# Gaeric/bevy-hikari

Measured on AMD Instinct MI355X. Metric: Mrays/sec + ms/frame @1080p 1spp; cornell & city scenes, 1/2/4/8 GPU, higher is better.
Workload: dtype f32

## Files before the change

### bevy-hikari_amd/csrc/hk_device.h

```cpp
#pragma once

#include <hip/hip_runtime.h>
#include <stdint.h>

#include "../../include/hk_math.h"
#include "../../include/hk_types.h"
#include "../../include/hikari_amd.h"
#include "../../include/hk_texture.h"

namespace hk {

struct f2 {
    float x, y;
};
struct f3 {
    float x, y, z;
};
struct f4 {
    float x, y, z, w;
};
#define HKD __device__ __forceinline__
HKD f2 mk2(float x, float y) { return f2{x, y}; }
HKD f3 mk3(float x, float y, float z) { return f3{x, y, z}; }
HKD f4 mk4(float x, float y, float z, float w) { return f4{x, y, z, w}; }
// ... 80 lines not shown
    const hk_node* asset_nodes;
    const hk_alias_entry* alias_table;
    const hk_instance* instances;
    const hk_node* instance_nodes;
    const hk_material* materials;
    const hk_node* emissive_nodes;
    const hk_emissive* emissives;
    uint32_t n_instances, n_instance_nodes, n_materials, n_emissive_nodes;
    const float4* blas_wide;
    const float4* tlas_wide;
    uint32_t bytes[SCENE_ARRAYS];
    const hk_texture_desc* textures;
    const uint32_t* texels;
    const float* texture_lut;
    uint32_t n_textures;
};

constexpr uint32_t LDS_SCENE_MAX = 32768;
constexpr uint32_t LDS_WORKGROUP_MAX = 65536;
enum : int { PLAN_LIGHT = 0, PLAN_GBUFFER = 1 };
__host__ __device__ constexpr bool plan_has(int plan, int k)
{
    return plan == PLAN_LIGHT ? k < 9 : (k == 0 || k == 1 || k == 4 || k == 9 || k == 10);
}
__host__ __device__ inline uint32_t stage_bytes(const uint32_t* bytes, int plan)
{
    uint32_t total = 0;
    for (int k = 0; k < 11; ++k)
        if (plan_has(plan, k)) total += (bytes[k] + 15u) & ~15u;
    return total;
// ... 631 lines not shown
{
    f4 r = mat4_mul(in.model, mk4(p.x, p.y, p.z, 1.0f));
    if (r.w == 1.0f) return mk3(r.x, r.y, r.z);
    return mk3(r.x / r.w, r.y / r.w, r.z / r.w);
}
HKD f3 local_to_world_normal(const hk_instance& in, f3 n)
{
    const float* m = in.inverse_transpose_model;
    f3 r;
    r.x = (m[0] * n.x + m[4] * n.y) + m[8] * n.z;
    r.y = (m[1] * n.x + m[5] * n.y) + m[9] * n.z;
    r.z = (m[2] * n.x + m[6] * n.y) + m[10] * n.z;
    return normalize(r);
}

constexpr int LANE_SLOTS = 5;
#ifdef HK_LANE_STATS
extern __device__ unsigned long long hk_lane_stats_dev[2 * LANE_SLOTS];
template <int SLOT = 0>
struct LaneStats {
    unsigned long long act = 0, its = 0;
    HKD void tick()
    {
        const unsigned long long m = __ballot(1);
        if ((uint32_t)__builtin_ctzll(m) == (threadIdx.x & 63u)) {
            act += (unsigned long long)__builtin_popcountll(m);
            its += 1;
        }
    }
    HKD ~LaneStats()
    {
        if (its) {
            atomicAdd(&hk_lane_stats_dev[2 * SLOT], act);
            atomicAdd(&hk_lane_stats_dev[2 * SLOT + 1], its);
        }
    }
};
#define HK_LANE_STATS_DECL LaneStats<0> lane_stats_
#define HK_LANE_STATS_TICK lane_stats_.tick()
#define HK_STAGE_STATS_DECL LaneStats<1> stage1_; LaneStats<2> stage2_; LaneStats<3> stage3_; LaneStats<4> stage4_
#define HK_STAGE_TICK(k) stage##k##_.tick()
#else
#define HK_LANE_STATS_DECL
#define HK_LANE_STATS_TICK
#define HK_STAGE_STATS_DECL
#define HK_STAGE_TICK(k)
#endif

template <bool ANY_HIT = true>
HKD Hit traverse_top(const Scene& sc, const Ray& ray, float max_distance, float early_distance, uint32_t exclude)
{
    Hit hit;
    hit.uv = mk2(0.0f, 0.0f);
    hit.distance = max_distance;
    hit.instance_index = HK_U32_MAX;
    hit.primitive_index = HK_U32_MAX;
    const hk_node* nodes = sc.instance_nodes;
    uint32_t count = sc.n_instance_nodes, index = 0u;
    Ray tr = ray;
    uint32_t top = 0u;
    uint32_t prim_offset = 0u, cur_instance = 0u;
    bool in_bottom = false, intersected = false;
    HK_LANE_STATS_DECL;
    while (index < count) {
        HK_LANE_STATS_TICK;
// ... 31 lines not shown
            }
        } else {
            const uint32_t instance_index = leaf_entry - HK_BVH_LEAF_FLAG;
            if (leaf_pass && (!ANY_HIT || instance_index != exclude)) {
                const hk_instance& in = sc.instances[instance_index];
                const uint32_t bot_count = in.mesh.node[1];
                prim_offset = in.mesh.primitive;
                cur_instance = instance_index;
                intersected = false;
                if (bot_count > 0u) {
                    in_bottom = true;
                    top = index;
                    nodes = sc.asset_nodes + in.mesh.node[0];
                    count = bot_count;
                    index = 0u;
                    tr.origin = world_to_local_point(in, ray.origin);
                    tr.direction = world_to_local_dir(in, ray.direction);
                    tr.inv_direction = inv(tr.direction);
                }
            }
        }
    }
    return hit;
}
HKD Hit traverse_top_closest(const Scene& sc, const Ray& ray)
{
    return traverse_top<false>(sc, ray, HK_F32_MAX, 0.0f, DONT_EXCLUDE);
}

constexpr int GB_STACK = 64;
constexpr int GB_STACK_LDS = 16;
constexpr int GB_DEEP_LDS = 8;
template <bool SHALLOW, int LVL = GB_STACK_LDS>
struct GbStackT {
    uint2* lds;
    uint32_t node[SHALLOW ? 1 : GB_STACK - LVL];
    float t[SHALLOW ? 1 : GB_STACK - LVL];
    int sp;
// ... 557 lines not shown
```

### bevy-hikari_amd/csrc/hk_kernels.hip

```cpp
#include <stdlib.h>
#include <mutex>
#include <type_traits>

#include "hk_device.h"
#include "hk_launch.h"

namespace hk {

#ifdef HK_LANE_STATS
__device__ unsigned long long hk_lane_stats_dev[2 * LANE_SLOTS];
#endif
bool lane_stats_take(unsigned long long out[2 * LANE_SLOTS], hipStream_t st)
{
#ifdef HK_LANE_STATS
    unsigned long long zero[2 * LANE_SLOTS] = {};
    if (hipStreamSynchronize(st) != hipSuccess) return false;
    if (hipMemcpyFromSymbol(out, HIP_SYMBOL(hk_lane_stats_dev), sizeof(zero)) != hipSuccess) return false;
    return hipMemcpyToSymbol(HIP_SYMBOL(hk_lane_stats_dev), zero, sizeof(zero)) == hipSuccess;
#else
    (void)st;
    for (int k = 0; k < 2 * LANE_SLOTS; ++k) out[k] = 0;
    return false;
#endif
}
// ... 639 lines not shown
}

template <bool VD, bool VE, int PARK>
HKD void fused_direct_pixel(const FrameArgs& A, const Scene& sc, const ChannelArgs& C0, const ChannelArgs& C1,
                            const DirectPixel& P, uint32_t& n_top, uint32_t& n_emitter)
{
    const uint32_t bg = bg_elide(C0, P.idx, P.pd.w < HK_F32_EPSILON);
    if (bg == BG_SKIP_OWN) {
        store_background_pair(C1, P.idx);
    } else if (bg == BG_STORE) {
        Surface surface;
        direct_body<false, true, VD, PARK>(A, sc, C0, P, n_top, n_emitter, &surface);
        direct_body<true, false, VE, PARK>(A, sc, C1, P, n_top, n_emitter, nullptr, &surface);
    }
}
template <bool LDS, bool VD, bool VE>
HKD void direct_fused_kernel(FrameArgs A, ChannelArgs C0, ChannelArgs C1)
{
    int32_t x, y;
    const bool active = tile_pixel<TRACE_ORDER>(A.F, A.F.s[0], A.F.s_row0, A.F.s_rows, x, y);
    PixelTexels tex;
    if (active) tex = load_pixel_texels(A, x, y);
    Scene sc;
    if constexpr (LDS) sc = stage_scene<PLAN_LIGHT>(A.sc, hk_lds_scene);
    else sc = A.sc;
    uint32_t n_top = 0, n_emitter = 0;
    if (active) fused_direct_pixel<VD, VE, !LDS>(A, sc, C0, C1, direct_pixel_of(A, x, y, tex), n_top, n_emitter);
    finish_counts(A, x, y, n_top, n_emitter);
}
template <bool LDS, bool VD, bool VE>
__global__ __launch_bounds__(256) void k_direct_fused(FrameArgs A, ChannelArgs C0, ChannelArgs C1)
{
    direct_fused_kernel<LDS, VD, VE>(A, C0, C1);
}
template <bool LDS, bool VD, bool VE = false>
__global__ __launch_bounds__(256) __attribute__((amdgpu_waves_per_eu(4, 8))) void k_direct_fused_w4(FrameArgs A, ChannelArgs C0,
                                                                                                   ChannelArgs C1)
{
    direct_fused_kernel<LDS, VD, VE>(A, C0, C1);
}

constexpr uint32_t CW_LONG_NODES = 16u;
constexpr int CW_WORDS = 10;
static_assert(CW_WORDS <= PARK_WORDS, "the batch rows fit the park columns");
HKD float* cw_area()
{
    __shared__ float cw[CW_WORDS * 256];
    return cw;
}
struct WalkRows {
    float* lds;
    uint32_t col;
    HKD float& operator[](int k) const { return lds[k * 256 + col]; }
    HKD uint32_t bits(int k) const { return __float_as_uint(lds[k * 256 + col]); }
// ... 535 lines not shown
template <bool MULTI, int STAGE = IND_ALL>
HKD bool indirect_body(const FrameArgs& A, const Scene& sc, const ChannelArgs& C, int32_t x, int32_t y, uint32_t& n_top,
                       uint32_t& n_emitter, const WfArgs* W = nullptr, uint32_t* key = nullptr, IndStash* stash = nullptr,
                       const PixelTexels* tex = nullptr)
{
    IndirectState I;
    bool ret;
    if (!indirect_begin<MULTI, STAGE>(A, sc, C, x, y, n_top, n_emitter, W, key, I, ret, stash, tex)) return ret;
    Hit sh;
    if (!MULTI && I.shadow)
        sh = traverse_top(sc, I.B.ray, I.B.cand.max_distance, I.B.cand.min_distance, I.B.cand.emissive_instance);
    indirect_end<MULTI>(A, sc, C, I, sh, stash);
    return true;
}

template <bool MULTI, bool LDS, bool CS = false>
__global__ __launch_bounds__(256) void k_indirect(FrameArgs A, ChannelArgs C)
{
    int32_t x, y;
    const bool active = tile_pixel<TRACE_ORDER>(A.F, A.F.s[0], A.F.s_row0, A.F.s_rows, x, y);
    constexpr bool PRE = !MULTI && !LDS && !CS;
    PixelTexels tex;
    if (PRE && active) tex = load_pixel_texels(A, x, y);
    Scene sc = A.sc;
    if constexpr (LDS) {
        sc = stage_scene<PLAN_LIGHT>(A.sc, hk_lds_scene);
    }
    uint32_t n_top = 0, n_emitter = 0;
    if constexpr (CS && !MULTI) {
        IndirectState I;
        bool ret = false;
        const bool live = active && indirect_begin<false>(A, sc, C, x, y, n_top, n_emitter, nullptr, nullptr, I, ret);
        Hit sh;
        compact_top_walks(sc, cw_area(), live && I.shadow, I.B.ray, I.B.cand.max_distance, I.B.cand.min_distance,
                          I.B.cand.emissive_instance, sh);
        if (live) indirect_end<false>(A, sc, C, I, sh);
    } else if (active) {
        __shared__ IndStash stash;
        indirect_body<MULTI>(A, sc, C, x, y, n_top, n_emitter, nullptr, nullptr, &stash, PRE ? &tex : nullptr);
    }
    finish_counts(A, x, y, n_top, n_emitter);
}
// ... 911 lines not shown
            if (emissive_lit) hipLaunchKernelGGL((k_direct<true, false, LDS, VAL>), g, dim3(256), lds, st, A, C);
            else if (big) hipLaunchKernelGGL((k_direct_lit_w4<LDS, VAL>), g, dim3(256), lds, st, A, C);
            else hipLaunchKernelGGL((k_direct<false, true, LDS, VAL>), g, dim3(256), lds, st, A, C);
        },
        lds != 0u, val);
}
template <bool LDS>
static void launch_fused_v(const FrameArgs& A, const ChannelArgs& C0, const ChannelArgs& C1, bool vd, bool ve, dim3 g,
                           uint32_t lds, hipStream_t st)
{
    const bool w4 = A.opt.fused_w4 != 0;
    if (!LDS && w4 && !ve && (A.opt.compact_emitter || A.opt.compact_shadow)) {
        dispatch([&](auto VD, auto CS) { hipLaunchKernelGGL((k_direct_fused_cw<VD, CS>), g, dim3(256), lds, st, A, C0, C1); },
                 vd, A.opt.compact_shadow != 0);
    } else if (w4 && (!LDS || !ve)) {
        dispatch([&](auto VD, auto VE) { hipLaunchKernelGGL((k_direct_fused_w4<LDS, VD, VE>), g, dim3(256), lds, st, A, C0, C1); },
                 vd, ve);
    } else {
        dispatch([&](auto VD, auto VE) { hipLaunchKernelGGL((k_direct_fused<LDS, VD, VE>), g, dim3(256), lds, st, A, C0, C1); },
                 vd, ve);
    }
}
void launch_direct_fused(const FrameArgs& A, const ChannelArgs& C0, const ChannelArgs& C1, hipStream_t st)
{
    dim3 g = tiles(A.F, A.F.s[0], A.F.s_rows);
    const uint32_t lds = lds_plan_bytes(A, PLAN_LIGHT, true);
    const bool vd = validation_frame(A.F.number, A.F.direct_validate_interval);
    const bool ve = validation_frame(A.F.number, A.F.emissive_validate_interval);
    if (lds) launch_fused_v<true>(A, C0, C1, vd, ve, g, lds, st);
    else launch_fused_v<false>(A, C0, C1, vd, ve, g, 0, st);
}
static uint32_t persist_grid(const void* kernel, uint32_t lds, const Frame& F)
// ... 31 lines not shown
}
void launch_indirect(const FrameArgs& A, const ChannelArgs& C, bool multi, hipStream_t st)
{
    dim3 g = tiles(A.F, A.F.s[0], A.F.s_rows);
    const uint32_t lds = lds_plan_bytes(A, PLAN_LIGHT, true);
    if (A.opt.persistent_indirect) {
        dispatch(
            [&](auto M, auto L) {
                const dim3 pg(persist_grid((const void*)k_indirect_persist<M, L>, lds, A.F));
                hipLaunchKernelGGL((k_indirect_persist<M, L>), pg, dim3(256), lds, st, A, C);
            },
            multi, lds != 0u);
        return;
    }
    dispatch(
        [&](auto L) {
            if (multi) hipLaunchKernelGGL((k_indirect<true, L>), g, dim3(256), lds, st, A, C);
            else if (A.opt.compact_shadow) hipLaunchKernelGGL((k_indirect<false, L, true>), g, dim3(256), lds, st, A, C);
            else hipLaunchKernelGGL((k_indirect<false, L>), g, dim3(256), lds, st, A, C);
        },
        lds != 0u);
}
uint32_t indirect_stash_bytes() { return (uint32_t)sizeof(IndStash); }
static_assert(LDS_SCENE_MAX + sizeof(IndStash) <= LDS_WORKGROUP_MAX, "staged scene + stash exceed a workgroup's LDS");
bool light_lds_direct(const FrameArgs& A) { return lds_plan_bytes(A, PLAN_LIGHT, false) != 0u; }
void launch_light_merged(const FrameArgs& A, const ChannelArgs& C0, const ChannelArgs& C1, const ChannelArgs& C2,
                         hipStream_t st)
{
    dim3 g = tiles(A.F, A.F.s[0], A.F.s_rows);
    g.z = 2u;
    const uint32_t scene = lds_plan_bytes(A, PLAN_LIGHT, true);
    const bool vd = validation_frame(A.F.number, A.F.direct_validate_interval);
    const bool ve = validation_frame(A.F.number, A.F.emissive_validate_interval);
    const uint32_t park = (vd || ve) ? (uint32_t)(PARK_WORDS * 256 * sizeof(float)) : 0u;
    const uint32_t ind = scene + (uint32_t)sizeof(IndStash);
    const uint32_t lds = ind > park ? ind : park;
// ... 251 lines not shown
```

### bevy-hikari_amd/csrc/hk_runtime.hip

```cpp
#include <hip/hip_runtime.h>

#include <algorithm>
#include <array>
#include <cmath>
#include <cstdio>
#include <cstring>
#include <map>
#include <set>
#include <string>
#include <vector>

#include "../../include/hikari_amd.h"
#include "hk_launch.h"

using namespace hk;

namespace {
constexpr int32_t BAND_HALO = 40;
constexpr size_t COUNTER_SPAN = (size_t)COUNTER_SHARDS * COUNTER_STRIDE;
constexpr size_t COUNTER_BYTES = 3 * COUNTER_SPAN * sizeof(unsigned long long);
constexpr size_t PERSIST_BYTES = (size_t)PERSIST_KINDS * PERSIST_LINES * PERSIST_LINE * sizeof(unsigned long long);

struct TimedLaunch {
    const char* name;
    hipEvent_t start, stop;
};

// ... 10 lines not shown
    OPT_SPATIAL_VIEW,
    OPT_BAND_FULL_WINDOWS,
    OPT_LEAF_COLLAPSE,
    OPT_GBUFFER_REUSE,
    OPT_LDS_SCENE,
    OPT_GBUFFER_STACK_FULL,
    OPT_GBUFFER_DEEP,
    OPT_GBUFFER_LDS_MAX_PX,
    OPT_DIRECT_W4_MIN_PX,
    OPT_FUSED_W4,
    OPT_PERSISTENT_INDIRECT,
    OPT_COMPACT_EMITTER,
    OPT_COMPACT_SHADOW,
    OPT_FSR_TILED,
    OPT_PRESENT_RUN,
    OPT_COUNT
};
struct OptDef {
    const char* key;
    double def, lo, hi;
};
constexpr OptDef OPTS[OPT_COUNT] = {
    {"pipeline_min_px", 1.2e6, 0.0, 1e12}, {"pipeline_heavy_min_px", 0.0, 0.0, 1e12},
    {"gbuffer_pipeline", 1, 0, 1},         {"tail_pipeline", 1, 0, 1},
    {"channel_streams", 1, 0, 1},          {"fuse", 1, 0, 1},              {"fuse_min_px", 1048576.0, 0.0, 1e12},
    {"merge", -1, -1, 1},                  {"bg_elision", 1, 0, 1},        {"spatial_view_planes", 1, 0, 1},
    {"band_full_windows", 0, 0, 1},        {"leaf_collapse", 1, 0, 1},     {"gbuffer_reuse", 1, 0, 1},
    {"lds_scene", 1, 0, 2},                {"gbuffer_stack_full", 0, 0, 1}, {"gbuffer_deep", 0, 0, 1},
    {"gbuffer_lds_max_px", 6e5, 0.0, 1e12},
    {"direct_w4_min_px", 4e5, 0.0, 1e12},  {"fused_w4", 1, 0, 1},          {"persistent_indirect", 0, 0, 1},
    {"compact_emitter", 0, 0, 1},          {"compact_shadow", 0, 0, 1},    {"fsr_tiled", 1, 0, 1},
    {"present_run", 1, 0, 1},
};

struct GSlot {
    float4* position = nullptr;
    uint32_t* normal = nullptr;
    float2* depth_gradient = nullptr;
    float2* instance_material = nullptr;
    float4* velocity_uv = nullptr;
    uint2* albedo = nullptr;
};

struct ScheduleState {
    bool gb_pending = false;
    bool gb_serial = true;
    bool post_pending = false;
// ... 153 lines not shown
        uint32_t vertex_need;
        uint32_t depth;
        uint32_t used = 0;
    };
    std::vector<MeshSlice> meshes;
    size_t cap[9] = {};
    size_t collapse_cap = 0;
    std::vector<float> emissive;
    uint32_t* blas_aux = nullptr;
    void* mesh_scratch = nullptr;
    size_t mesh_bytes = 0;
    float* prev_models = nullptr;
    bool models_dirty = false;
    bool velocity_zero = true;
    bool has_scene = false;
    uchar4* noise = nullptr;
    bool has_noise = false;
    hk_texture_desc* tex_desc = nullptr;
    uint32_t* texels = nullptr;
    float* tex_lut = nullptr;
    uint32_t n_textures = 0;

    uint32_t S[2] = {0, 0}, s[2] = {0, 0};
    float ratio = 1.0f;
    int32_t S_row0 = 0, S_rows = 0, s_row0 = 0, s_rows = 0;
    int32_t core_row0 = 0, core_rows = 0;
    int32_t halo = BAND_HALO;
    int32_t stripe_n = 0, stripe_k = 0;
    bool albedo_fresh = false;
    bool sized = false;
// ... 209 lines not shown
{
    if (!c->event_pool.empty()) {
        hipEvent_t e = c->event_pool.back();
        c->event_pool.pop_back();
        return e;
    }
    hipEvent_t e = nullptr;
    (void)hipEventCreate(&e);
    return e;
}

void lane_stats_account(hk_ctx* c, const char* name, hipStream_t st)
{
    unsigned long long v[2 * LANE_SLOTS];
    if (!lane_stats_take(v, st)) return;
    static const char* const stage[LANE_SLOTS] = {"", "/neighbour", "/march_tap", "/record_tests", "/merge"};
    for (int slot = 0; slot < LANE_SLOTS; ++slot) {
        if (!v[2 * slot + 1]) continue;
        const std::string key = std::string(name) + stage[slot];
        size_t k = 0;
        for (; k < c->lane_names.size(); ++k)
            if (c->lane_names[k] == key) break;
        if (k == c->lane_names.size()) {
            c->lane_names.push_back(key);
            c->lane_act.push_back(0);
            c->lane_its.push_back(0);
        }
        c->lane_act[k] += v[2 * slot];
        c->lane_its[k] += v[2 * slot + 1];
    }
}
// ... 64 lines not shown
    A.sc.instances = (const hk_instance*)c->buf[4];
    A.sc.instance_nodes = c->walk_nodes[1];
    A.sc.materials = (const hk_material*)c->buf[6];
    A.sc.emissive_nodes = (const hk_node*)c->buf[7];
    A.sc.emissives = (const hk_emissive*)c->buf[8];
    A.sc.n_instances = c->count[4];
    A.sc.n_instance_nodes = c->count[5];
    A.sc.n_materials = c->count[6];
    A.sc.n_emissive_nodes = c->count[7];
    A.sc.blas_wide = c->blas_wide;
    A.sc.tlas_wide = c->tlas_wide;
    A.sc.textures = c->tex_desc;
    A.sc.texels = c->texels;
    A.sc.texture_lut = c->tex_lut;
    A.sc.n_textures = c->n_textures;
    scene_array_bytes(c->count, A.sc.bytes);
    Frame& F = A.F;
    hk_settings def;
    hk_settings_default(&def);
    if (!st) st = &def;
    F.number = in ? in->frame_number : 0u;
    F.direct_validate_interval = st->direct_validate_interval;
    F.emissive_validate_interval = st->emissive_validate_interval;
    F.max_temporal_reuse_count = st->max_temporal_reuse_count;
    F.max_spatial_reuse_count = st->max_spatial_reuse_count;
    F.indirect_bounces = st->indirect_bounces;
    F.temporal_reuse = st->temporal_reuse;
    F.max_reservoir_lifetime = st->max_reservoir_lifetime;
    F.max_indirect_luminance = st->max_indirect_luminance;
    F.upscale_ratio = c->ratio;
// ... 402 lines not shown
    if (lds_levels) *lds_levels = (uint32_t)GB_STACK_LDS;
    return HK_OK;
}

int hk_scene_upload(hk_ctx* c, const hk_scene_desc* d)
{
    if (!c || !d) return HK_ERR_INVALID;
    (void)hipSetDevice(c->device);
    HK_TRY(c->sch.gb_serialize(true));
    const hk_array* arr[9] = {&d->vertices, &d->primitives, &d->asset_nodes, &d->alias_table, &d->instances,
                              &d->instance_nodes, &d->materials, &d->emissive_nodes, &d->emissives};
    const size_t* elem = SCENE_ELEM;
    if (d->instances.count == 0 || d->materials.count == 0)
        return fail(c, HK_ERR_INVALID, "scene needs at least one instance and one material");
    c->gen++;
    for (int i = 0; i < 9; ++i)
        if (arr[i]->count && !arr[i]->data) return fail(c, HK_ERR_INVALID, "scene array with count but no data");
    HK_HIP(c, hipStreamSynchronize(c->stream));
    for (int i = 0; i < 9; ++i) {
        release(c->buf[i]);
        size_t bytes = staged_alloc_bytes(arr[i]->count, elem[i]);
        HK_HIP(c, hipMalloc(&c->buf[i], bytes));
        HK_HIP(c, hipMemset(c->buf[i], 0, bytes));
        if (arr[i]->count) HK_HIP(c, hipMemcpy(c->buf[i], arr[i]->data, arr[i]->count * elem[i], hipMemcpyHostToDevice));
        c->count[i] = arr[i]->count;
        c->cap[i] = arr[i]->count ? arr[i]->count : 1;
    }
    c->emissive.resize(4 * (size_t)d->materials.count);
    for (uint32_t k = 0; k < d->materials.count; ++k)
        std::memcpy(&c->emissive[4 * (size_t)k], ((const hk_material*)d->materials.data)[k].emissive, 16);
// ... 51 lines not shown
                             c->stream));
    HK_HIP(c, hipMemcpyAsync(c->walk_nodes[1], c->buf[5], (size_t)n_tlas * sizeof(hk_node), hipMemcpyDeviceToDevice,
                             c->stream));
    if (c->on(OPT_LEAF_COLLAPSE)) {
        launch_collapse_leaves(c->walk_nodes[0], n_blas, d_aux + n_blas, d_aux + 2 * (size_t)n_blas, c->collapse_scratch,
                               c->stream);
        launch_collapse_leaves(c->walk_nodes[1], n_tlas, nullptr, nullptr, c->collapse_scratch, c->stream);
    }
    HK_HIP(c, hipGetLastError());
    release(c->prev_models);
    HK_HIP(c, hipMalloc(&c->prev_models, (size_t)d->instances.count * 64));
    HK_HIP(c, hipMemcpy2DAsync(c->prev_models, 64, (const char*)c->buf[4] + offsetof(hk_instance, model),
                               sizeof(hk_instance), 64, d->instances.count, hipMemcpyDeviceToDevice, c->stream));
    c->models_dirty = false;
    HK_HIP(c, hipStreamSynchronize(c->stream));
    c->has_scene = true;
    return HK_OK;
}

struct MeshLevels {
    const uint32_t* device;
    std::vector<uint32_t> slice;
};

struct SetChange {
    const hk_instance_desc* set = nullptr;
    const hk_material* materials = nullptr;
    uint32_t counts[9] = {};
    std::vector<uint32_t> slice;
    std::vector<hk_ctx::MeshSlice> fresh;
// ... 165 lines not shown
    const size_t need = std::max<size_t>(1, std::max(c->count[2], counts[5]));
    if (need > c->collapse_cap) {
        const size_t cap = grown(need, c->collapse_cap);
        if (!fresh((void**)&c->collapse_scratch, cap * 4)) return fail(c, HK_ERR_HIP, "hk_set_instances: out of device memory");
        c->collapse_cap = cap;
    }
    return HK_OK;
}

static int rebuild_instances(hk_ctx* c, const float* models, const float* local_aabbs, uint32_t count, hipStream_t st,
                             const MeshLevels* ml, const SetChange* set = nullptr)
{
    HK_TRY(c->sch.gb_join(st));
    HK_TRY(c->sch.gb_serialize(false));
    c->gen++;
    struct Moved {
        float* p = nullptr;
        ~Moved() { release(p); }
    } old_prev;
    const uint32_t n_before = c->count[4];
    if (set) {
        HK_TRY(reserve_set(c, set->counts, &old_prev.p));
        if (!set->fresh.empty()) {
            const uint32_t n_blas = c->count[2];
            for (const hk_ctx::MeshSlice& f : set->fresh) {
                const hk_mesh_index& x = f.index;
                const uint32_t value[3] = {x.primitive, x.node[0], x.node[1]};
                std::vector<uint32_t> row(x.node[1]);
                for (int k = 0; k < 3; ++k) {
                    std::fill(row.begin(), row.end(), value[k]);
// ... 96 lines not shown
    HK_HIP(c, hipStreamSynchronize(st));
    if (ml) {
        for (size_t k = 0; k < levels.size(); ++k) c->meshes[ml->slice[k]].depth = levels[k];
        c->gb_blas_depth = 0;
        for (const hk_ctx::MeshSlice& s : c->meshes)
            if (s.used) c->gb_blas_depth = std::max(c->gb_blas_depth, s.depth);
    }
    if (ml || set) c->gb_stack_need = flags[1] + c->gb_blas_depth;
    if (set && (flags[2] != m || flags[3] != n_alias))
        return fail(c, HK_ERR_HIP, "hk_set_instances: the device counted " + std::to_string(flags[2]) + " emitters and " +
                                       std::to_string(flags[3]) + " alias entries, the host " + std::to_string(m) +
                                       " and " + std::to_string(n_alias));
    if (flags[0]) return fail(c, HK_ERR_INVALID, "singular instance transform");
    c->gb_stack_need = flags[1] + c->gb_blas_depth;
    c->models_dirty = true;
    return HK_OK;
}

static int update_args_ok(hk_ctx* c, uint32_t count, const char* who)
{
    if (!c->has_scene) return fail(c, HK_ERR_STATE, "no scene uploaded (hk_scene_upload)");
    if (count != c->count[4]) return fail(c, HK_ERR_INVALID, std::string(who) + " needs every instance, in upload order");
    if (c->count[5] != 3u * count - 2u || (c->count[8] && c->count[7] != 3u * c->count[8] - 2u))
        return fail(c, HK_ERR_STATE, "scene BVHs are not bvh-0.7.1 flattened (3n - 2 nodes); cannot rebuild");
    return HK_OK;
}

int hk_update_instances(hk_ctx* c, const float* models, const float* local_aabbs, uint32_t count, void* stream)
{
    if (!c || !models || !local_aabbs) return HK_ERR_INVALID;
// ... 129 lines not shown
    }
    SetChange change;
    std::string why;
    const int rc = plan_instance_set(c->count, c->meshes, materials ? emissive.data() : c->emissive.data(), set, count,
                                     SliceReader{nullptr, c}, &change, &why);
    if (rc != HK_OK) return fail(c, rc, "hk_set_instances: " + why);
    change.materials = materials;
    return rebuild_instances(c, models, local_aabbs, count, pick(c, stream), nullptr, &change);
}

int hk_scene_counts(const hk_ctx* c, uint32_t counts[9])
{
    if (!c || !counts) return HK_ERR_INVALID;
    if (!c->has_scene) return HK_ERR_STATE;
    std::memcpy(counts, c->count, sizeof(c->count));
    return HK_OK;
}

int hk_instance_set_counts(const hk_scene_desc* d, const hk_instance_desc* set, uint32_t count,
                           const hk_material* materials, uint32_t counts[9])
{
    if (!d || !set || !counts || !scene_desc_ok(d)) return HK_ERR_INVALID;
    const uint32_t before[9] = {d->vertices.count,  d->primitives.count,     d->asset_nodes.count,
                                d->alias_table.count, d->instances.count,    d->instance_nodes.count,
                                d->materials.count, d->emissive_nodes.count, d->emissives.count};
    std::vector<hk_ctx::MeshSlice> known;
    std::set<std::array<uint32_t, 4>> seen;
    const hk_instance* inst = (const hk_instance*)d->instances.data;
    for (uint32_t k = 0; k < d->instances.count; ++k) {
        const hk_mesh_index& m = inst[k].mesh;
// ... 1304 lines not shown
```

### bevy-hikari_amd/csrc/hk_scene.cpp

```cpp
#include "../../include/hikari_scene.h"

#include <algorithm>
#include <cmath>
#include <cstring>
#include <limits>
#include <string>
#include <vector>

namespace {

struct V3 {
    float x, y, z;
};
static inline V3 v3(float x, float y, float z) { return V3{x, y, z}; }
static inline V3 operator+(V3 a, V3 b) { return v3(a.x + b.x, a.y + b.y, a.z + b.z); }
static inline V3 operator-(V3 a, V3 b) { return v3(a.x - b.x, a.y - b.y, a.z - b.z); }
static inline V3 operator*(V3 a, float s) { return v3(a.x * s, a.y * s, a.z * s); }
static inline V3 vmin(V3 a, V3 b) { return v3(std::fmin(a.x, b.x), std::fmin(a.y, b.y), std::fmin(a.z, b.z)); }
static inline V3 vmax(V3 a, V3 b) { return v3(std::fmax(a.x, b.x), std::fmax(a.y, b.y), std::fmax(a.z, b.z)); }
static inline float dot(V3 a, V3 b) { return a.x * b.x + a.y * b.y + a.z * b.z; }
static inline V3 cross(V3 a, V3 b)
{
    return v3(a.y * b.z - b.y * a.z, a.z * b.x - b.z * a.x, a.x * b.y - b.x * a.y);
}
// ... 470 lines not shown
int hks_get_desc(const hks_scene* s, hk_scene_desc* out)
{
    if (!s || !out) return HK_ERR_INVALID;
    out->vertices = hk_array{s->vertices.data(), (uint32_t)s->vertices.size()};
    out->primitives = hk_array{s->primitives.data(), (uint32_t)s->primitives.size()};
    out->asset_nodes = hk_array{s->asset_nodes.data(), (uint32_t)s->asset_nodes.size()};
    out->alias_table = hk_array{s->alias_table.data(), (uint32_t)s->alias_table.size()};
    out->instances = hk_array{s->gpu_instances.data(), (uint32_t)s->gpu_instances.size()};
    out->instance_nodes = hk_array{s->instance_nodes.data(), (uint32_t)s->instance_nodes.size()};
    out->materials = hk_array{s->materials.data(), (uint32_t)s->materials.size()};
    out->emissive_nodes = hk_array{s->emissive_nodes.data(), (uint32_t)s->emissive_nodes.size()};
    out->emissives = hk_array{s->emissives.data(), (uint32_t)s->emissives.size()};
    return HK_OK;
}

}
```

### bevy-hikari_amd/hikari_amd/__init__.py

```python
from . import _abi
from ._abi import HikariError
from .plugin import (HikariPlugin, HikariRenderer, PLAN_GBUFFER, PLAN_LIGHT, RESERVOIR_DTYPE, instance_descs,
                     instance_set_counts, scene_gbuffer_stack, scene_indirect_lds, scene_stage_bytes)
from .scene import (AmbientLight, Camera, DirectionalLight, Mesh, Scene, StandardMaterial, Texture, Transform,
                    frame_inputs, jitter_mode, load_glb, load_noise, make_lights, plane_mesh, texture_array, uv_sphere_mesh)
from .settings import HikariSettings, HikariUniversalSettings, PresentFormat, Taa, Upscale

__all__ = [
    "HikariError", "HikariPlugin", "HikariRenderer", "RESERVOIR_DTYPE", "AmbientLight", "Camera", "DirectionalLight",
    "Mesh", "Scene", "StandardMaterial", "Texture", "texture_array", "Transform", "frame_inputs", "jitter_mode", "load_glb", "load_noise", "make_lights",
    "plane_mesh", "uv_sphere_mesh", "scene_stage_bytes", "scene_indirect_lds", "scene_gbuffer_stack", "instance_descs", "instance_set_counts", "PLAN_LIGHT", "PLAN_GBUFFER", "HikariSettings", "HikariUniversalSettings", "PresentFormat", "Taa", "Upscale", "_abi",
]
```

### bevy-hikari_amd/hikari_amd/_abi.py

```python
from __future__ import annotations

import ctypes as C
import os
from pathlib import Path

HERE = Path(__file__).resolve().parent
LIB_PATH = Path(os.environ["HK_LIB"]) if os.environ.get("HK_LIB") else HERE / "libhikari_amd.so"

HK_OK = 0
HK_ERR_INVALID = -1
HK_ERR_HIP = -2
HK_ERR_STATE = -3
HK_ERR_NO_DEVICE = -4

RESERVOIR_BUFFERS = 10

OUT_ALBEDO = 0
OUT_VARIANCE = (1, 2, 3)
OUT_RENDER = (4, 5, 6)
OUT_DENOISED = (7, 8, 9)
OUT_TONE_MAPPED = 10
OUT_GBUF_POSITION = 11
OUT_GBUF_NORMAL = 12
OUT_GBUF_DEPTH_GRADIENT = 13
# ... 155 lines not shown
        "hk_render_gbuffer": (i32, [vp, C.POINTER(hk_frame_inputs), vp]),
        "hk_set_gbuffer_plane": (i32, [vp, i32, vp, C.c_size_t, i32, vp]),
        "hk_render_frame": (i32, [vp, C.POINTER(hk_settings), C.POINTER(hk_frame_inputs), vp]),
        "hk_denoise": (i32, [vp, C.POINTER(hk_settings), C.POINTER(hk_frame_inputs), vp]),
        "hk_tone_sum": (i32, [vp, C.POINTER(hk_settings), vp]),
        "hk_accumulate": (i32, [vp, i32, vp]),
        "hk_post_process": (i32, [vp, C.POINTER(hk_settings), C.POINTER(hk_frame_inputs), vp]),
        "hk_set_fsr1_sharpness": (i32, [vp, C.c_float]),
        "hk_present": (i32, [vp, C.POINTER(hk_settings), C.POINTER(hk_present_target), vp]),
        "hk_present_info": (i32, [vp] + [C.POINTER(u32)] * 4),
        "hk_get_present": (i32, [vp, vp, C.c_size_t, i32, vp]),
        "hk_update_instances": (i32, [vp, vp, vp, u32, vp]),
        "hk_update_meshes": (i32, [vp, C.POINTER(hk_mesh_update), u32, vp, vp, u32, vp]),
        "hk_set_instances": (i32, [vp, C.POINTER(hk_instance_desc), vp, vp, u32, vp, vp]),
        "hk_scene_counts": (i32, [vp, C.POINTER(u32)]),
        "hk_instance_set_counts": (i32, [C.POINTER(hk_scene_desc), C.POINTER(hk_instance_desc), u32, vp, C.POINTER(u32)]),
        "hk_read_scene_array": (i32, [vp, i32, vp, C.c_size_t]),
        "hk_resolve_accumulation": (i32, [vp, vp]),
        "hk_output_info": (i32, [vp, i32, C.POINTER(u32), C.POINTER(u32), C.POINTER(u32)]),
        "hk_get_output": (i32, [vp, i32, vp, C.c_size_t, i32, vp]),
        "hk_output_device_ptr": (vp, [vp, i32]),
        "hk_sync": (i32, [vp, vp]),
        "hk_set_wavefront": (i32, [vp, i32]),
        "hk_lane_stats": (i32, [vp, C.POINTER(C.c_char_p), C.POINTER(C.c_uint64), C.POINTER(C.c_uint64), i32]),
        "hk_dump_reservoirs": (i32, [vp, i32, vp, C.c_size_t, vp]),
        "hk_load_reservoirs": (i32, [vp, i32, vp, C.c_size_t, vp]),
        "hk_reset_counters": (i32, [vp, vp]),
        "hk_read_counters": (i32, [vp, C.POINTER(hk_counters), vp]),
        "hk_enable_kernel_timing": (i32, [vp, i32]),
        "hk_kernel_timing": (i32, [vp, C.POINTER(C.c_char_p), C.POINTER(C.c_float), i32]),
        "hk_set_kernel_timing_interval": (i32, [vp, u32]),
        "hk_trace": (i32, [vp, vp, vp, vp, vp, u32, vp, i32, vp]),
        "hk_selftest_f16": (i32, [vp, vp, u32, vp]),
        "hk_selftest_div": (i32, [vp, C.c_float, u32, u32, C.POINTER(C.c_uint64)]),
        "hk_selftest_rcp": (i32, [vp, u32, u32, C.POINTER(C.c_uint64)]),
        "hk_selftest_count": (i32, [vp, vp, u32, C.POINTER(C.c_uint64)]),
        "hks_create": (vp, []),
        "hks_destroy": (None, [vp]),
        "hks_last_error": (C.c_char_p, [vp]),
        "hks_add_mesh": (i32, [vp, vp, vp, vp, u32, vp, u32, i32]),
        "hks_add_material": (i32, [vp, vp]),
        "hks_add_instance": (i32, [vp, u32, u32, vp]),
        "hks_build": (i32, [vp, i32]),
        "hks_get_desc": (i32, [vp, C.POINTER(hk_scene_desc)]),
    }
    for name, (res, args) in sig.items():
        f = getattr(L, name)
        f.restype = res
        f.argtypes = args
    _lib = L
    return L


EXPORTED_SYMBOLS = [
    "hk_abi_version", "hk_create", "hk_destroy", "hk_last_error", "hk_settings_default", "hk_set_option",
    "hk_get_option", "hk_option_name", "hk_scene_upload", "hk_scene_stage_bytes", "hk_scene_indirect_lds",
    "hk_scene_gbuffer_stack",
    "hk_set_noise", "hk_texture_upload", "hk_resize", "hk_resize_striped", "hk_set_band_halo", "hk_band_info", "hk_band_window_grow", "hk_reservoir_rows", "hk_resize_tile", "hk_tile_info", "hk_copy_output_rect", "hk_copy_output_rows", "hk_render_gbuffer", "hk_set_gbuffer_plane", "hk_render_frame",
    "hk_denoise", "hk_tone_sum", "hk_update_instances", "hk_update_meshes", "hk_set_instances", "hk_scene_counts", "hk_instance_set_counts", "hk_read_scene_array", "hk_post_process", "hk_set_fsr1_sharpness", "hk_present", "hk_present_info", "hk_get_present", "hk_accumulate", "hk_resolve_accumulation", "hk_output_info", "hk_get_output", "hk_output_device_ptr", "hk_sync", "hk_set_wavefront", "hk_lane_stats", "hk_dump_reservoirs",
    "hk_load_reservoirs", "hk_reset_counters", "hk_read_counters", "hk_enable_kernel_timing", "hk_kernel_timing", "hk_set_kernel_timing_interval",
    "hk_trace", "hk_selftest_f16", "hk_selftest_div", "hk_selftest_rcp", "hk_selftest_count", "hks_create", "hks_destroy", "hks_last_error", "hks_add_mesh", "hks_add_material",
    "hks_add_instance", "hks_build", "hks_get_desc",
]


def gpu_visible() -> bool:
    return bool(os.environ.get("HIP_VISIBLE_DEVICES", "x")) and Path("/dev/kfd").exists()
```

### bevy-hikari_amd/hikari_amd/plugin.py

```python
from __future__ import annotations

import ctypes as C
from typing import Optional

import numpy as np

from . import _abi
from .scene import Scene, load_noise, texture_array
from .settings import HikariSettings, HikariUniversalSettings, PresentFormat

RESERVOIR_DTYPE = np.dtype([("radiance", "<u4", 2), ("random", "<u4", 2), ("visible_position", "<f4", 4),
                            ("sample_position", "<f4", 4), ("visible_normal", "<u4"), ("sample_normal", "<u4"),
                            ("reservoir", "<u4", 2)])
assert RESERVOIR_DTYPE.itemsize == 64


def _stream(stream):
    if stream is None or isinstance(stream, (int, C.c_void_p)):
        return stream
    raise TypeError(f"stream must be None or an integer hipStream_t handle, not {type(stream).__name__}")


def _check(ctx, rc: int, what: str) -> None:
    if rc != 0:
# ... 13 lines not shown


def scene_indirect_lds(scene):
    desc = scene if isinstance(scene, _abi.hk_scene_desc) else (scene.desc if scene.desc is not None else scene.build())
    s, t, lim = C.c_uint32(), C.c_uint32(), C.c_uint32()
    _check(None, _abi.lib().hk_scene_indirect_lds(C.byref(desc), C.byref(s), C.byref(t), C.byref(lim)),
           "hk_scene_indirect_lds")
    return s.value, t.value, lim.value


def scene_gbuffer_stack(scene):
    desc = scene if isinstance(scene, _abi.hk_scene_desc) else (scene.desc if scene.desc is not None else scene.build())
    n, lv = C.c_uint32(), C.c_uint32()
    _check(None, _abi.lib().hk_scene_gbuffer_stack(C.byref(desc), C.byref(n), C.byref(lv)), "hk_scene_gbuffer_stack")
    return n.value, lv.value


def instance_descs(scene: Scene, previous=None):
    n = len(scene.instances)
    if previous is not None and len(previous) != n:
        raise ValueError("previous needs one entry per instance")
    out = (_abi.hk_instance_desc * max(1, n))()
    slices = {}
    for k, (mesh, mat, _) in enumerate(scene.instances):
        if mesh not in slices:
            v, pr, n0, nc = scene.mesh_index(mesh)
            slices[mesh] = _abi.hk_mesh_index(v, pr, (C.c_uint32 * 2)(n0, nc))
        p = None if previous is None else previous[k]
        out[k] = _abi.hk_instance_desc(slices[mesh], int(mat), _abi.HK_INSTANCE_NEW if p is None else int(p))
    return out
# ... 176 lines not shown
                      local_aabbs=None) -> None:
        m = np.ascontiguousarray(scene.instance_models() if models is None else models, np.float32).reshape(-1, 16)
        a = np.ascontiguousarray(scene.instance_local_aabbs() if local_aabbs is None else local_aabbs,
                                 np.float32).reshape(-1, 6)
        if len(m) != len(a) or len(m) != len(scene.instances):
            raise ValueError("models and local_aabbs need one record per instance")
        mats = material_records(scene) if materials else None
        _check(self.ctx, self._L.hk_set_instances(self.ctx, instance_descs(scene, previous), m.ctypes.data, a.ctypes.data,
                                                  len(m), mats, _stream(stream)), "hk_set_instances")

    def scene_counts(self) -> list:
        out = (C.c_uint32 * 9)()
        _check(self.ctx, self._L.hk_scene_counts(self.ctx, out), "hk_scene_counts")
        return list(out)

    def scene_array(self, array: int, dtype, count: int) -> np.ndarray:
        out = np.empty(count, dtype)
        _check(self.ctx, self._L.hk_read_scene_array(self.ctx, array, out.ctypes.data, out.nbytes),
               "hk_read_scene_array")
        return out

    def post_process(self, settings: _abi.hk_settings, inputs: _abi.hk_frame_inputs, stream=None) -> None:
        _check(self.ctx, self._L.hk_post_process(self.ctx, C.byref(settings), C.byref(inputs), _stream(stream)),
               "hk_post_process")

    def set_fsr1_sharpness(self, sharpness: float) -> None:
        _check(self.ctx, self._L.hk_set_fsr1_sharpness(self.ctx, float(sharpness)), "hk_set_fsr1_sharpness")

    def present(self, settings, width: int, height: int, format="rgba8_srgb", viewport=None, input: int = -1,
                dst_ptr: Optional[int] = None, pitch: int = 0, stream=None):
# ... 177 lines not shown
```

### include/hikari_amd.h

```cpp
#ifndef HIKARI_AMD_H
#define HIKARI_AMD_H

#include <stddef.h>
#include <stdint.h>
#include "hk_types.h"
#include "hk_texture.h"

#ifdef __cplusplus
extern "C" {
#endif

#define HK_ABI_VERSION 3

enum {
    HK_OK = 0,
    HK_ERR_INVALID = -1,
    HK_ERR_HIP = -2,
    HK_ERR_STATE = -3,
    HK_ERR_NO_DEVICE = -4,
};

typedef struct hk_ctx hk_ctx;

typedef struct hk_array {
// ... 120 lines not shown
    const float* positions;
    const float* normals;
} hk_mesh_update;
int hk_update_meshes(hk_ctx* ctx, const hk_mesh_update* meshes, uint32_t mesh_count, const float* models,
                     const float* local_aabbs, uint32_t count, void* stream);

#define HK_INSTANCE_NEW 0xFFFFFFFFu
typedef struct hk_instance_desc {
    hk_mesh_index mesh;
    uint32_t material;
    uint32_t previous;
} hk_instance_desc;
int hk_set_instances(hk_ctx* ctx, const hk_instance_desc* set, const float* models, const float* local_aabbs,
                     uint32_t count, const hk_material* materials, void* stream);
int hk_scene_counts(const hk_ctx* ctx, uint32_t counts[9]);
int hk_instance_set_counts(const hk_scene_desc* uploaded, const hk_instance_desc* set, uint32_t count,
                           const hk_material* materials, uint32_t counts[9]);
int hk_scene_stage_bytes(const hk_scene_desc* scene, int plan, uint32_t* bytes, uint32_t* limit);
int hk_scene_indirect_lds(const hk_scene_desc* scene, uint32_t* stash, uint32_t* total, uint32_t* limit);
int hk_scene_gbuffer_stack(const hk_scene_desc* scene, uint32_t* need, uint32_t* lds_levels);
int hk_read_scene_array(hk_ctx* ctx, int array, void* dst, size_t bytes);

int hk_post_process(hk_ctx* ctx, const hk_settings* settings, const hk_frame_inputs* inputs, void* stream);
int hk_set_fsr1_sharpness(hk_ctx* ctx, float sharpness);

enum { HK_PRESENT_RGBA8_SRGB = 0, HK_PRESENT_BGRA8_SRGB = 1, HK_PRESENT_RGBA16F = 2 };
typedef struct hk_present_target {
    void*    data;
    uint32_t width, height;
    uint32_t pitch;
// ... 73 lines not shown
```

### include/hikari_scene.h

```cpp
#ifndef HIKARI_SCENE_H
#define HIKARI_SCENE_H

#include <stdint.h>
#include "hikari_amd.h"

#ifdef __cplusplus
extern "C" {
#endif

typedef struct hks_scene hks_scene;

enum { HKS_TRIANGLE_LIST = 0, HKS_TRIANGLE_STRIP = 1 };

hks_scene* hks_create(void);
void hks_destroy(hks_scene* scene);
const char* hks_last_error(const hks_scene* scene);

int hks_add_mesh(hks_scene* scene, const float* positions, const float* normals, const float* uvs,
                 uint32_t vertex_count, const uint32_t* indices, uint32_t index_count, int topology);
int hks_add_material(hks_scene* scene, const hk_material* material);
int hks_add_instance(hks_scene* scene, uint32_t mesh, uint32_t material, const float* model);

int hks_build(hks_scene* scene, int buckets);
int hks_get_desc(const hks_scene* scene, hk_scene_desc* out);

#ifdef __cplusplus
}
#endif

#endif
```

Measured before the change: 10740.

## Hoist instance transform out of traversal when all instances share one matrix

When every instance has an identical transform, the kernel computes the ray's local-space origin and direction once per ray instead of on each descent into a bottom BVH. The host detects the shared-transform case, exposes it as an option, and dispatches specialised direct and indirect kernel variants with the flag fixed at compile time. This removes repeated matrix-vector work and reciprocal computation per instance entry. The cost is extra kernel instantiations and register pressure from holding both the world-space and local-space rays.

```diff
diff --git a/bevy-hikari_amd/csrc/hk_device.h b/bevy-hikari_amd/csrc/hk_device.h
--- a/bevy-hikari_amd/csrc/hk_device.h
+++ b/bevy-hikari_amd/csrc/hk_device.h
@@ -118,6 +118,7 @@
     const uint32_t* texels;
     const float* texture_lut;
     uint32_t n_textures;
+    uint32_t shared_xform;
 };
 
 constexpr uint32_t LDS_SCENE_MAX = 32768;
@@ -779,7 +780,7 @@
     return normalize(r);
 }
 
-constexpr int LANE_SLOTS = 5;
+constexpr int LANE_SLOTS = 6;
 #ifdef HK_LANE_STATS
 extern __device__ unsigned long long hk_lane_stats_dev[2 * LANE_SLOTS];
 template <int SLOT = 0>
@@ -801,19 +802,21 @@
         }
     }
 };
-#define HK_LANE_STATS_DECL LaneStats<0> lane_stats_
+#define HK_LANE_STATS_DECL LaneStats<0> lane_stats_; LaneStats<5> entry_stats_
 #define HK_LANE_STATS_TICK lane_stats_.tick()
+#define HK_ENTRY_STATS_TICK entry_stats_.tick()
 #define HK_STAGE_STATS_DECL LaneStats<1> stage1_; LaneStats<2> stage2_; LaneStats<3> stage3_; LaneStats<4> stage4_
 #define HK_STAGE_TICK(k) stage##k##_.tick()
 #else
 #define HK_LANE_STATS_DECL
 #define HK_LANE_STATS_TICK
+#define HK_ENTRY_STATS_TICK
 #define HK_STAGE_STATS_DECL
 #define HK_STAGE_TICK(k)
 #endif
 
-template <bool ANY_HIT = true>
-HKD Hit traverse_top(const Scene& sc, const Ray& ray, float max_distance, float early_distance, uint32_t exclude)
+template <bool ANY_HIT>
+HKD Hit traverse_top_general(const Scene& sc, const Ray& ray, float max_distance, float early_distance, uint32_t exclude)
 {
     Hit hit;
     hit.uv = mk2(0.0f, 0.0f);
@@ -875,6 +878,7 @@
                     nodes = sc.asset_nodes + in.mesh.node[0];
                     count = bot_count;
                     index = 0u;
+                    HK_ENTRY_STATS_TICK;
                     tr.origin = world_to_local_point(in, ray.origin);
                     tr.direction = world_to_local_dir(in, ray.direction);
                     tr.inv_direction = inv(tr.direction);
@@ -883,6 +887,91 @@
         }
     }
     return hit;
+}
+template <bool ANY_HIT>
+HKD Hit traverse_top_shared(const Scene& sc, const Ray& ray, float max_distance, float early_distance, uint32_t exclude)
+{
+    Hit hit;
+    hit.uv = mk2(0.0f, 0.0f);
+    hit.distance = max_distance;
+    hit.instance_index = HK_U32_MAX;
+    hit.primitive_index = HK_U32_MAX;
+    const hk_node* nodes = sc.instance_nodes;
+    uint32_t count = sc.n_instance_nodes, index = 0u;
+    Ray local;
+    {
+        const hk_instance& in0 = sc.instances[0];
+        local.origin = world_to_local_point(in0, ray.origin);
+        local.direction = world_to_local_dir(in0, ray.direction);
+        local.inv_direction = inv(local.direction);
+    }
+    uint32_t top = 0u;
+    uint32_t prim_offset = 0u, cur_instance = 0u;
+    bool in_bottom = false, intersected = false;
+    HK_LANE_STATS_DECL;
+    while (index < count) {
+        HK_LANE_STATS_TICK;
+        Ray tr;
+        tr.origin = in_bottom ? local.origin : ray.origin;
+        tr.direction = local.direction;
+        tr.inv_direction = in_bottom ? local.inv_direction : ray.inv_direction;
+        bool leaf_pass;
+        uint32_t leaf_entry;
+        index = walk_step<WALK_STEPS>(nodes, index, count, tr, hit.distance, leaf_pass, leaf_entry);
+        if (in_bottom) {
+            bool stop = false;
+            if (leaf_pass) {
+                const uint32_t primitive_index = prim_offset + leaf_entry - HK_BVH_LEAF_FLAG;
+                f3 a, b, c;
+                load_triangle(sc.primitives, primitive_index, a, b, c);
+                f2 uv;
+                const float d = intersects_triangle(local, a, b, c, uv);
+                if (d < hit.distance) {
+                    hit.distance = d;
+                    hit.uv = uv;
+                    hit.primitive_index = primitive_index;
+                    intersected = true;
+                    if constexpr (ANY_HIT) stop = d < early_distance;
+                }
+            }
+            if (stop || index >= count) {
+                in_bottom = false;
+                nodes = sc.instance_nodes;
+                count = sc.n_instance_nodes;
+                index = top;
+                if (intersected) {
+                    hit.instance_index = cur_instance;
+                    if constexpr (ANY_HIT) {
+                        if (hit.distance < early_distance) return hit;
+                    }
+                }
+            }
+        } else {
+            const uint32_t instance_index = leaf_entry - HK_BVH_LEAF_FLAG;
+            if (leaf_pass && (!ANY_HIT || instance_index != exclude)) {
+                const hk_instance& in = sc.instances[instance_index];
+                const uint32_t bot_count = in.mesh.node[1];
+                prim_offset = in.mesh.primitive;
+                cur_instance = instance_index;
+                intersected = false;
+                if (bot_count > 0u) {
+                    in_bottom = true;
+                    top = index;
+                    nodes = sc.asset_nodes + in.mesh.node[0];
+                    count = bot_count;
+                    index = 0u;
+                    HK_ENTRY_STATS_TICK;
+                }
+            }
+        }
+    }
+    return hit;
+}
+template <bool ANY_HIT = true>
+HKD Hit traverse_top(const Scene& sc, const Ray& ray, float max_distance, float early_distance, uint32_t exclude)
+{
+    if (sc.shared_xform) return traverse_top_shared<ANY_HIT>(sc, ray, max_distance, early_distance, exclude);
+    return traverse_top_general<ANY_HIT>(sc, ray, max_distance, early_distance, exclude);
 }
 HKD Hit traverse_top_closest(const Scene& sc, const Ray& ray)
 {
diff --git a/bevy-hikari_amd/csrc/hk_kernels.hip b/bevy-hikari_amd/csrc/hk_kernels.hip
--- a/bevy-hikari_amd/csrc/hk_kernels.hip
+++ b/bevy-hikari_amd/csrc/hk_kernels.hip
@@ -677,7 +677,12 @@
         direct_body<true, false, VE, PARK>(A, sc, C1, P, n_top, n_emitter, nullptr, &surface);
     }
 }
-template <bool LDS, bool VD, bool VE>
+template <int SX>
+HKD void fix_shared_xform(Scene& sc)
+{
+    if constexpr (SX >= 0) sc.shared_xform = (uint32_t)SX;
+}
+template <bool LDS, bool VD, bool VE, int SX = -1>
 HKD void direct_fused_kernel(FrameArgs A, ChannelArgs C0, ChannelArgs C1)
 {
     int32_t x, y;
@@ -687,6 +692,7 @@
     Scene sc;
     if constexpr (LDS) sc = stage_scene<PLAN_LIGHT>(A.sc, hk_lds_scene);
     else sc = A.sc;
+    fix_shared_xform<SX>(sc);
     uint32_t n_top = 0, n_emitter = 0;
     if (active) fused_direct_pixel<VD, VE, !LDS>(A, sc, C0, C1, direct_pixel_of(A, x, y, tex), n_top, n_emitter);
     finish_counts(A, x, y, n_top, n_emitter);
@@ -696,11 +702,11 @@
 {
     direct_fused_kernel<LDS, VD, VE>(A, C0, C1);
 }
-template <bool LDS, bool VD, bool VE = false>
+template <bool LDS, bool VD, bool VE = false, bool SX = false>
 __global__ __launch_bounds__(256) __attribute__((amdgpu_waves_per_eu(4, 8))) void k_direct_fused_w4(FrameArgs A, ChannelArgs C0,
                                                                                                    ChannelArgs C1)
 {
-    direct_fused_kernel<LDS, VD, VE>(A, C0, C1);
+    direct_fused_kernel<LDS, VD, VE, SX ? 1 : 0>(A, C0, C1);
 }
 
 constexpr uint32_t CW_LONG_NODES = 16u;
@@ -1266,7 +1272,7 @@
     return true;
 }
 
-template <bool MULTI, bool LDS, bool CS = false>
+template <bool MULTI, bool LDS, bool CS = false, int SX = -1>
 __global__ __launch_bounds__(256) void k_indirect(FrameArgs A, ChannelArgs C)
 {
     int32_t x, y;
@@ -1278,6 +1284,7 @@
     if constexpr (LDS) {
         sc = stage_scene<PLAN_LIGHT>(A.sc, hk_lds_scene);
     }
+    fix_shared_xform<SX>(sc);
     uint32_t n_top = 0, n_emitter = 0;
     if constexpr (CS && !MULTI) {
         IndirectState I;
@@ -2219,8 +2226,8 @@
         dispatch([&](auto VD, auto CS) { hipLaunchKernelGGL((k_direct_fused_cw<VD, CS>), g, dim3(256), lds, st, A, C0, C1); },
                  vd, A.opt.compact_shadow != 0);
     } else if (w4 && (!LDS || !ve)) {
-        dispatch([&](auto VD, auto VE) { hipLaunchKernelGGL((k_direct_fused_w4<LDS, VD, VE>), g, dim3(256), lds, st, A, C0, C1); },
-                 vd, ve);
+        dispatch([&](auto VD, auto VE, auto SX) { hipLaunchKernelGGL((k_direct_fused_w4<LDS, VD, VE, SX>), g, dim3(256), lds, st, A, C0, C1); },
+                 vd, ve, A.sc.shared_xform != 0u);
     } else {
         dispatch([&](auto VD, auto VE) { hipLaunchKernelGGL((k_direct_fused<LDS, VD, VE>), g, dim3(256), lds, st, A, C0, C1); },
                  vd, ve);
@@ -2282,12 +2289,12 @@
         return;
     }
     dispatch(
-        [&](auto L) {
+        [&](auto L, auto SX) {
             if (multi) hipLaunchKernelGGL((k_indirect<true, L>), g, dim3(256), lds, st, A, C);
             else if (A.opt.compact_shadow) hipLaunchKernelGGL((k_indirect<false, L, true>), g, dim3(256), lds, st, A, C);
-            else hipLaunchKernelGGL((k_indirect<false, L>), g, dim3(256), lds, st, A, C);
+            else hipLaunchKernelGGL((k_indirect<false, L, false, SX ? 1 : 0>), g, dim3(256), lds, st, A, C);
         },
-        lds != 0u);
+        lds != 0u, A.sc.shared_xform != 0u);
 }
 uint32_t indirect_stash_bytes() { return (uint32_t)sizeof(IndStash); }
 static_assert(LDS_SCENE_MAX + sizeof(IndStash) <= LDS_WORKGROUP_MAX, "staged scene + stash exceed a workgroup's LDS");
diff --git a/bevy-hikari_amd/csrc/hk_runtime.hip b/bevy-hikari_amd/csrc/hk_runtime.hip
--- a/bevy-hikari_amd/csrc/hk_runtime.hip
+++ b/bevy-hikari_amd/csrc/hk_runtime.hip
@@ -11,6 +11,7 @@
 #include <vector>
 
 #include "../../include/hikari_amd.h"
+#include "../../include/hikari_scene.h"
 #include "hk_launch.h"
 
 using namespace hk;
@@ -51,6 +52,7 @@
     OPT_COMPACT_SHADOW,
     OPT_FSR_TILED,
     OPT_PRESENT_RUN,
+    OPT_SHARED_XFORM,
     OPT_COUNT
 };
 struct OptDef {
@@ -67,7 +69,7 @@
     {"gbuffer_lds_max_px", 6e5, 0.0, 1e12},
     {"direct_w4_min_px", 4e5, 0.0, 1e12},  {"fused_w4", 1, 0, 1},          {"persistent_indirect", 0, 0, 1},
     {"compact_emitter", 0, 0, 1},          {"compact_shadow", 0, 0, 1},    {"fsr_tiled", 1, 0, 1},
-    {"present_run", 1, 0, 1},
+    {"present_run", 1, 0, 1},              {"shared_xform", 1, 0, 1},
 };
 
 struct GSlot {
@@ -251,6 +253,7 @@
     bool models_dirty = false;
     bool velocity_zero = true;
     bool has_scene = false;
+    bool shared_transform = false;
     uchar4* noise = nullptr;
     bool has_noise = false;
     hk_texture_desc* tex_desc = nullptr;
@@ -490,7 +493,8 @@
 {
     unsigned long long v[2 * LANE_SLOTS];
     if (!lane_stats_take(v, st)) return;
-    static const char* const stage[LANE_SLOTS] = {"", "/neighbour", "/march_tap", "/record_tests", "/merge"};
+    static const char* const stage[LANE_SLOTS] = {"", "/neighbour", "/march_tap", "/record_tests", "/merge",
+                                                    "/instance_entry"};
     for (int slot = 0; slot < LANE_SLOTS; ++slot) {
         if (!v[2 * slot + 1]) continue;
         const std::string key = std::string(name) + stage[slot];
@@ -585,6 +589,7 @@
     A.sc.texels = c->texels;
     A.sc.texture_lut = c->tex_lut;
     A.sc.n_textures = c->n_textures;
+    A.sc.shared_xform = c->shared_transform && c->on(OPT_SHARED_XFORM);
     scene_array_bytes(c->count, A.sc.bytes);
     Frame& F = A.F;
     hk_settings def;
@@ -1017,6 +1022,7 @@
     if (d->instances.count == 0 || d->materials.count == 0)
         return fail(c, HK_ERR_INVALID, "scene needs at least one instance and one material");
     c->gen++;
+    c->shared_transform = false;
     for (int i = 0; i < 9; ++i)
         if (arr[i]->count && !arr[i]->data) return fail(c, HK_ERR_INVALID, "scene array with count but no data");
     HK_HIP(c, hipStreamSynchronize(c->stream));
@@ -1098,6 +1104,11 @@
                                sizeof(hk_instance), 64, d->instances.count, hipMemcpyDeviceToDevice, c->stream));
     c->models_dirty = false;
     HK_HIP(c, hipStreamSynchronize(c->stream));
+    {
+        std::vector<float> itm(16 * (size_t)d->instances.count);
+        for (uint32_t k = 0; k < d->instances.count; ++k) std::memcpy(&itm[16 * (size_t)k], inst[k].inverse_transpose_model, 64);
+        c->shared_transform = hks_shared_transform(itm.data(), d->instances.count) != 0;
+    }
     c->has_scene = true;
     return HK_OK;
 }
@@ -1293,6 +1304,7 @@
     HK_TRY(c->sch.gb_join(st));
     HK_TRY(c->sch.gb_serialize(false));
     c->gen++;
+    c->shared_transform = false;
     struct Moved {
         float* p = nullptr;
         ~Moved() { release(p); }
@@ -1419,6 +1431,7 @@
     if (flags[0]) return fail(c, HK_ERR_INVALID, "singular instance transform");
     c->gb_stack_need = flags[1] + c->gb_blas_depth;
     c->models_dirty = true;
+    c->shared_transform = hks_shared_transform(models, n) != 0;
     return HK_OK;
 }
 
@@ -1578,6 +1591,14 @@
     if (!c || !counts) return HK_ERR_INVALID;
     if (!c->has_scene) return HK_ERR_STATE;
     std::memcpy(counts, c->count, sizeof(c->count));
+    return HK_OK;
+}
+
+int hk_scene_shared_transform(const hk_ctx* c, int32_t* shared)
+{
+    if (!c || !shared) return HK_ERR_INVALID;
+    if (!c->has_scene) return HK_ERR_STATE;
+    *shared = c->shared_transform ? 1 : 0;
     return HK_OK;
 }
 
diff --git a/bevy-hikari_amd/csrc/hk_scene.cpp b/bevy-hikari_amd/csrc/hk_scene.cpp
--- a/bevy-hikari_amd/csrc/hk_scene.cpp
+++ b/bevy-hikari_amd/csrc/hk_scene.cpp
@@ -508,4 +508,12 @@
     return HK_OK;
 }
 
-}
+int hks_shared_transform(const float* matrices, uint32_t n)
+{
+    if (!matrices || n == 0) return 0;
+    for (uint32_t k = 1; k < n; ++k)
+        if (std::memcmp(matrices, matrices + 16 * (size_t)k, 64) != 0) return 0;
+    return 1;
+}
+
+}
diff --git a/bevy-hikari_amd/hikari_amd/__init__.py b/bevy-hikari_amd/hikari_amd/__init__.py
--- a/bevy-hikari_amd/hikari_amd/__init__.py
+++ b/bevy-hikari_amd/hikari_amd/__init__.py
@@ -1,7 +1,7 @@
 from . import _abi
 from ._abi import HikariError
 from .plugin import (HikariPlugin, HikariRenderer, PLAN_GBUFFER, PLAN_LIGHT, RESERVOIR_DTYPE, instance_descs,
-                     instance_set_counts, scene_gbuffer_stack, scene_indirect_lds, scene_stage_bytes)
+                     instance_set_counts, scene_gbuffer_stack, scene_indirect_lds, scene_stage_bytes, shared_transform)
 from .scene import (AmbientLight, Camera, DirectionalLight, Mesh, Scene, StandardMaterial, Texture, Transform,
                     frame_inputs, jitter_mode, load_glb, load_noise, make_lights, plane_mesh, texture_array, uv_sphere_mesh)
 from .settings import HikariSettings, HikariUniversalSettings, PresentFormat, Taa, Upscale
@@ -9,5 +9,5 @@
 __all__ = [
     "HikariError", "HikariPlugin", "HikariRenderer", "RESERVOIR_DTYPE", "AmbientLight", "Camera", "DirectionalLight",
     "Mesh", "Scene", "StandardMaterial", "Texture", "texture_array", "Transform", "frame_inputs", "jitter_mode", "load_glb", "load_noise", "make_lights",
-    "plane_mesh", "uv_sphere_mesh", "scene_stage_bytes", "scene_indirect_lds", "scene_gbuffer_stack", "instance_descs", "instance_set_counts", "PLAN_LIGHT", "PLAN_GBUFFER", "HikariSettings", "HikariUniversalSettings", "PresentFormat", "Taa", "Upscale", "_abi",
+    "plane_mesh", "uv_sphere_mesh", "scene_stage_bytes", "scene_indirect_lds", "scene_gbuffer_stack", "shared_transform", "instance_descs", "instance_set_counts", "PLAN_LIGHT", "PLAN_GBUFFER", "HikariSettings", "HikariUniversalSettings", "PresentFormat", "Taa", "Upscale", "_abi",
 ]
diff --git a/bevy-hikari_amd/hikari_amd/_abi.py b/bevy-hikari_amd/hikari_amd/_abi.py
--- a/bevy-hikari_amd/hikari_amd/_abi.py
+++ b/bevy-hikari_amd/hikari_amd/_abi.py
@@ -193,6 +193,7 @@
         "hk_update_meshes": (i32, [vp, C.POINTER(hk_mesh_update), u32, vp, vp, u32, vp]),
         "hk_set_instances": (i32, [vp, C.POINTER(hk_instance_desc), vp, vp, u32, vp, vp]),
         "hk_scene_counts": (i32, [vp, C.POINTER(u32)]),
+        "hk_scene_shared_transform": (i32, [vp, C.POINTER(i32)]),
         "hk_instance_set_counts": (i32, [C.POINTER(hk_scene_desc), C.POINTER(hk_instance_desc), u32, vp, C.POINTER(u32)]),
         "hk_read_scene_array": (i32, [vp, i32, vp, C.c_size_t]),
         "hk_resolve_accumulation": (i32, [vp, vp]),
@@ -222,6 +223,7 @@
         "hks_add_instance": (i32, [vp, u32, u32, vp]),
         "hks_build": (i32, [vp, i32]),
         "hks_get_desc": (i32, [vp, C.POINTER(hk_scene_desc)]),
+        "hks_shared_transform": (i32, [vp, u32]),
     }
     for name, (res, args) in sig.items():
         f = getattr(L, name)
@@ -239,7 +241,7 @@
     "hk_denoise", "hk_tone_sum", "hk_update_instances", "hk_update_meshes", "hk_set_instances", "hk_scene_counts", "hk_instance_set_counts", "hk_read_scene_array", "hk_post_process", "hk_set_fsr1_sharpness", "hk_present", "hk_present_info", "hk_get_present", "hk_accumulate", "hk_resolve_accumulation", "hk_output_info", "hk_get_output", "hk_output_device_ptr", "hk_sync", "hk_set_wavefront", "hk_lane_stats", "hk_dump_reservoirs",
     "hk_load_reservoirs", "hk_reset_counters", "hk_read_counters", "hk_enable_kernel_timing", "hk_kernel_timing", "hk_set_kernel_timing_interval",
     "hk_trace", "hk_selftest_f16", "hk_selftest_div", "hk_selftest_rcp", "hk_selftest_count", "hks_create", "hks_destroy", "hks_last_error", "hks_add_mesh", "hks_add_material",
-    "hks_add_instance", "hks_build", "hks_get_desc",
+    "hks_add_instance", "hks_build", "hks_get_desc", "hk_scene_shared_transform", "hks_shared_transform",
 ]
 
 
diff --git a/bevy-hikari_amd/hikari_amd/plugin.py b/bevy-hikari_amd/hikari_amd/plugin.py
--- a/bevy-hikari_amd/hikari_amd/plugin.py
+++ b/bevy-hikari_amd/hikari_amd/plugin.py
@@ -51,6 +51,11 @@
     n, lv = C.c_uint32(), C.c_uint32()
     _check(None, _abi.lib().hk_scene_gbuffer_stack(C.byref(desc), C.byref(n), C.byref(lv)), "hk_scene_gbuffer_stack")
     return n.value, lv.value
+
+
+def shared_transform(models) -> bool:
+    m = np.ascontiguousarray(models, np.float32).reshape(-1, 16)
+    return bool(_abi.lib().hks_shared_transform(m.ctypes.data if len(m) else None, len(m)))
 
 
 def instance_descs(scene: Scene, previous=None):
@@ -257,6 +262,11 @@
         _check(self.ctx, self._L.hk_scene_counts(self.ctx, out), "hk_scene_counts")
         return list(out)
 
+    def scene_shared_transform(self) -> bool:
+        out = C.c_int32()
+        _check(self.ctx, self._L.hk_scene_shared_transform(self.ctx, C.byref(out)), "hk_scene_shared_transform")
+        return bool(out.value)
+
     def scene_array(self, array: int, dtype, count: int) -> np.ndarray:
         out = np.empty(count, dtype)
         _check(self.ctx, self._L.hk_read_scene_array(self.ctx, array, out.ctypes.data, out.nbytes),
diff --git a/include/hikari_amd.h b/include/hikari_amd.h
--- a/include/hikari_amd.h
+++ b/include/hikari_amd.h
@@ -158,6 +158,7 @@
 int hk_set_instances(hk_ctx* ctx, const hk_instance_desc* set, const float* models, const float* local_aabbs,
                      uint32_t count, const hk_material* materials, void* stream);
 int hk_scene_counts(const hk_ctx* ctx, uint32_t counts[9]);
+int hk_scene_shared_transform(const hk_ctx* ctx, int32_t* shared);
 int hk_instance_set_counts(const hk_scene_desc* uploaded, const hk_instance_desc* set, uint32_t count,
                            const hk_material* materials, uint32_t counts[9]);
 int hk_scene_stage_bytes(const hk_scene_desc* scene, int plan, uint32_t* bytes, uint32_t* limit);
diff --git a/include/hikari_scene.h b/include/hikari_scene.h
--- a/include/hikari_scene.h
+++ b/include/hikari_scene.h
@@ -24,6 +24,8 @@
 int hks_build(hks_scene* scene, int buckets);
 int hks_get_desc(const hks_scene* scene, hk_scene_desc* out);
 
+int hks_shared_transform(const float* matrices, uint32_t n);
+
 #ifdef __cplusplus
 }
 #endif
```

Result: faster. 11040, median of 6 (+2.8%).
